# e-c-k-e-r/tortoise-tts

Hardware: AMD Instinct MI355X
Metric: audio-sec/wall-sec (RTF^-1), 16 AR candidates x 80 DDIM steps (higher is better)
Workload: dtype bf16; 1 GPU; configs[1]: 1 utterance/GPU, 64 text tokens, 16 AR candidates x 250 mel tokens (KV-cached decode), latent pass on 16 candidates, 80 DDIM steps with cond-free guidance at T=1088 (11.6 s audio); candidates=16, ddim_steps=80, mel_frames=1088, parallelism=single GPU, small_models=False, vocoder_in_step=False

## Files before the change

tortoise_tts_amd/csrc/ar.hip:

```cpp
#include "ttk_common.h"
#include "ttk_conv.h"

using namespace ttk;

namespace {

struct ARLayer {
	float *ln1_g, *ln1_b, *ln2_g, *ln2_b;
	Mat attn, proj, fc, proj2;
};

__global__ void k_build_prefill_emb(const float* cond, int Bc, const int64_t* text, int Tt, int B, int d,
									const float* text_emb, const float* text_pos, const float* mel_emb, const float* mel_pos,
									int start_text, int stop_text, int start_mel, float* out, const int64_t* prompt = nullptr, int prompt_rows = 0, int n_in = 0) {
	const int S = Tt + 4 + n_in;
	const int64_t idx = (int64_t)blockIdx.x * blockDim.x + threadIdx.x;
	const int d4 = d / 4;
	if (idx >= (int64_t)B * S * d4) return;
	const int c = (int)(idx % d4) * 4;
	const int64_t row = idx / d4;
	const int b = (int)(row / S), s = (int)(row - (int64_t)b * S);
	float4 v;
	if (s == 0) {
		v = *(const float4*)(cond + (int64_t)(Bc == 1 ? 0 : b) * d + c);
// ... 1 lines not shown
		const int j = s - (Tt + 3);
		const int64_t tok = j == 0 ? start_mel : prompt[(int64_t)(prompt_rows == 1 ? 0 : b) * n_in + j - 1];
		const float4 e = *(const float4*)(mel_emb + tok * d + c), w = *(const float4*)(mel_pos + (int64_t)j * d + c);
		v = make_float4(e.x + w.x, e.y + w.y, e.z + w.z, e.w + w.w);
	} else {
		const int j = s - 1;
		const int64_t tok = j == 0 ? start_text : (j == Tt + 1 ? stop_text : text[j - 1]);
		const float4 e = *(const float4*)(text_emb + tok * d + c), w = *(const float4*)(text_pos + (int64_t)j * d + c);
		v = make_float4(e.x + w.x, e.y + w.y, e.z + w.z, e.w + w.w);
	}
	*(float4*)(out + row * d + c) = v;
}

__global__ void k_build_latent_emb(const float* cond, const int64_t* text, int Tt, const int64_t* codes, int M, int B, int d,
								   const float* text_emb, const float* text_pos, const float* mel_emb, const float* mel_pos,
								   int start_text, int stop_text, int start_mel, int stop_mel, float* out) {
	const int S = Tt + M + 5;
	const int64_t idx = (int64_t)blockIdx.x * blockDim.x + threadIdx.x;
	const int d4 = d / 4;
	if (idx >= (int64_t)B * S * d4) return;
	const int c = (int)(idx % d4) * 4;
	const int64_t row = idx / d4;
	const int b = (int)(row / S), s = (int)(row - (int64_t)b * S);
	float4 v;
	if (s == 0) {
		v = *(const float4*)(cond + (int64_t)b * d + c);
	} else if (s < Tt + 3) {
		const int j = s - 1;
		const int64_t tok = j == 0 ? start_text : (j == Tt + 1 ? stop_text : text[(int64_t)b * Tt + j - 1]);
		const float4 e = *(const float4*)(text_emb + tok * d + c), w = *(const float4*)(text_pos + (int64_t)j * d + c);
		v = make_float4(e.x + w.x, e.y + w.y, e.z + w.z, e.w + w.w);
	} else {
		const int j = s - (Tt + 3);
		const int64_t tok = j == 0 ? start_mel : (j == M + 1 ? stop_mel : codes[(int64_t)b * M + j - 1]);
		const float4 e = *(const float4*)(mel_emb + tok * d + c), w = *(const float4*)(mel_pos + (int64_t)j * d + c);
		v = make_float4(e.x + w.x, e.y + w.y, e.z + w.z, e.w + w.w);
	}
	*(float4*)(out + row * d + c) = v;
}

__global__ void k_build_score_targets(const int64_t* text, int Tt, int stop_text, const int64_t* codes, int M, int stop_mel, int B, int64_t* tgt_text, int64_t* tgt_mel) {
	const int64_t idx = (int64_t)blockIdx.x * blockDim.x + threadIdx.x;
	const int64_t nt = (int64_t)B * (Tt + 2), nm = (int64_t)B * (M + 2);
	if (idx < nt) {
		const int b = (int)(idx / (Tt + 2)), j = (int)(idx - (int64_t)b * (Tt + 2));
		tgt_text[idx] = j < Tt ? text[(int64_t)b * Tt + j] : stop_text;
	} else if (idx < nt + nm) {
		const int64_t i = idx - nt;
		const int b = (int)(i / (M + 2)), j = (int)(i - (int64_t)b * (M + 2));
		tgt_mel[i] = j < M ? codes[(int64_t)b * M + j] : stop_mel;
	}
}

// ... 21 lines not shown
	void *attn_out, *hbuf;
	void* x_frag = nullptr;
	int poison = 0;
	int frag_rows = 0;
	int shared_rows = 0;
	const int64_t* rng_args = nullptr; const int64_t* rng_draws = nullptr; float* rng_q = nullptr;
	int* d_health = nullptr;
	float* ring_base = nullptr; const int64_t* ring_idx = nullptr; int64_t ring_stride = 0;
	int64_t* d_ring = nullptr;
	int lnfold = 1;
	int lean = 1;
	WsBuf ws_x, ws_a, ws_qkv, ws_ao, ws_h;
	WsBuf ws_score;
	int B = 0, P = 0, k = 0, ready = 0;
	int Pmax = 0;
	~ttk_ar() { attn_pos_slot_release(pos_slot); }
};

static int poison_scratch(ttk_ar* h, hipStream_t s) {
	if (!h->poison) return TTK_OK;
	for (WsBuf* w : {&h->ws_x, &h->ws_a, &h->ws_qkv, &h->ws_ao, &h->ws_h, &h->ws_score})
		if (w->p) TTK_HIP(hipMemsetAsync(w->p, 0xFF, w->cap, s));
	return TTK_OK;
}

static int dense_forward(ttk_ar* h, float* x, int B, int S, bool write_kv, hipStream_t s, int kv_row0 = 0, int kv_t0 = 0) {
	const int d = h->cfg.model_dim, H = h->cfg.heads, dt = h->dt;
	const int rows = B * S;
	TTK_TRY(h->ws_a.reserve((size_t)rows * d * h->es));
	TTK_TRY(h->ws_qkv.reserve((size_t)rows * 3 * d * h->es));
	TTK_TRY(h->ws_ao.reserve((size_t)rows * d * h->es));
	TTK_TRY(h->ws_h.reserve((size_t)rows * 4 * d * h->es));
	for (int l = 0; l < h->cfg.layers; ++l) {
		const ARLayer& L = h->L[l];
		launch_layernorm(dt, x, d, rows, d, L.ln1_g, L.ln1_b, nullptr, nullptr, h->ws_a.p, d, 0, s);
		launch_gemm(dt, dense_gemm(h->ws_a.p, d, L.attn, rows, h->ws_qkv.p, 0), s);
		if (write_kv) {
			const size_t row0 = (size_t)kv_row0 * H * h->cfg.max_ctx * 64;
			char* kc = (char*)h->kc + ((size_t)l * h->kv_layer_stride + row0) * h->es;
			char* vc = (char*)h->vc + ((size_t)l * h->kv_layer_stride + row0) * h->es;
			launch_kv_scatter(dt, h->ws_qkv.p, B, S, H, kc, vc, h->cfg.max_ctx, s, kv_t0);
		}
		AttnParams a = {};
		a.qkv = h->ws_qkv.p; a.ld = 3 * d; a.q_off = 0; a.k_off = d; a.v_off = 2 * d; a.head_stride = 64;
		a.out = h->ws_ao.p; a.ldo = d; a.nb = B; a.T = S; a.H = H; a.causal = 1; a.bias = nullptr; a.scale = 0.125f;
		launch_attn_fwd(dt, a, s);
		gemm_plain(dt, h->ws_ao.p, d, L.proj, rows, x, x, 1, s);
		launch_layernorm(dt, x, d, rows, d, L.ln2_g, L.ln2_b, nullptr, nullptr, h->ws_a.p, d, 0, s);
		GemmParams fc = dense_gemm(h->ws_a.p, d, L.fc, rows, h->ws_h.p, 0);
		fc.act = ACT_GELU_NEW;
		launch_gemm(dt, fc, s);
		gemm_plain(dt, h->ws_h.p, 4 * d, L.proj2, rows, x, x, 1, s);
	}
	return TTK_OK;
}

namespace ttk {

int skinny_waves(int role, bool ln_prologue, int dt, int d) {
	if (d < 1024 || role == DR_HEAD) return 4;
	if (ln_prologue || dt == DT_F32) return 8;
// ... 71 lines not shown
		TTK_TRY(decode_launch(ctx, proj, B, s));
		DecodeLaunch fc = {DR_FC, &L.fc, 4 * d, d, h->x_frag, L.ln2_g, L.ln2_b};
		fc.out_T = h->hbuf; fc.x = h->x; fc.ldx = d;
		TTK_TRY(decode_launch(ctx, fc, B, s));
		DecodeLaunch proj2 = {DR_PROJ2, &L.proj2, d, 4 * d, h->hbuf};
		proj2.out_f32 = h->x; proj2.out_T = xf;
		TTK_TRY(decode_launch(ctx, proj2, B, s));
	}
	if (h->ring_base && !hidden_out) launch_layernorm(dt, h->x, d, B, d, h->lnf_g, h->lnf_b, h->fn_g, h->fn_b, h->attn_out, d, 0, s, 1, nullptr, h->ring_idx, h->ring_stride, h->d_ring);
	else launch_layernorm(dt, h->x, d, B, d, h->lnf_g, h->lnf_b, h->fn_g, h->fn_b, h->attn_out, d, 0, s, 1, hidden_out);
	DecodeLaunch head = {DR_HEAD, &h->head, c.number_mel_codes, d, h->attn_out};
	head.out_f32 = logits_out; head.bump = true; head.d_pos = h->d_pos;
	return decode_launch(ctx, head, B, s);
}

extern "C" {

int ttk_ar_create(ttk_ar** out, const ttk_ar_config* cfg, const ttk_weight_view* w, int n_w) {
	TTK_REQUIRE(out && cfg && w, TTK_E_ARG, "ttk_ar_create: null argument");
	TTK_REQUIRE(cfg->model_dim % 64 == 0 && cfg->heads * 64 == cfg->model_dim, TTK_E_ARG,
				"ttk_ar_create: head_dim must be 64 (model_dim %d, heads %d)", cfg->model_dim, cfg->heads);
	TTK_REQUIRE(cfg->model_dim <= 2048, TTK_E_ARG, "ttk_ar_create: model_dim %d > 2048 unsupported", cfg->model_dim);
	TTK_REQUIRE(cfg->dtype == TTK_F32 || cfg->dtype == TTK_BF16 || cfg->dtype == TTK_F16 || cfg->dtype == TTK_FP8W, TTK_E_ARG, "ttk_ar_create: bad dtype %d", cfg->dtype);
	TTK_REQUIRE(cfg->max_batch >= 1 && cfg->max_batch <= (cfg->dtype == TTK_F32 ? 32 : 64), TTK_E_ARG,
				"ttk_ar_create: max_batch %d out of range", cfg->max_batch);
	TTK_REQUIRE(cfg->max_ctx >= 8, TTK_E_ARG, "ttk_ar_create: max_ctx %d too small", cfg->max_ctx);
	{
		const int kdt = kernel_dtype(cfg->dtype), d = cfg->model_dim;
		for (int B = 1; B <= cfg->max_batch; ++B) {
			const int mt = decode_row_tiles(B);
// ... 64 lines not shown
	for (int B = 1; B <= cfg->max_batch; ++B)
		if (16 * decode_row_tiles(B) > h->frag_rows) { set_error("ttk_ar_create: %d rows would request %d fragment rows, %d allocated", B, 16 * decode_row_tiles(B), h->frag_rows); return TTK_E_STATE; }
	TTK_TRY(h->arena.alloc(&h->attn_out, frag_rows * d * h->es));
	if (hipMemset(h->attn_out, 0, frag_rows * d * h->es) != hipSuccess) return TTK_E_HIP;
	TTK_TRY(h->arena.alloc(&h->hbuf, frag_rows * 4 * d * h->es));
	if (hipMemset(h->hbuf, 0, frag_rows * 4 * d * h->es) != hipSuccess) return TTK_E_HIP;
	TTK_TRY(h->arena.alloc(&h->x_frag, frag_rows * d * h->es));
	if (hipMemset(h->x_frag, 0, frag_rows * d * h->es) != hipSuccess) return TTK_E_HIP;
	{
		const char* ep = getenv("TTK_DEBUG_POISON");
		h->poison = ep && atoi(ep) != 0;
		const char* el = getenv("TTK_AR_LNFOLD");
		h->lnfold = el ? (atoi(el) != 0) : 1;
		const char* eg = getenv("TTK_AR_LEAN");
		h->lean = eg ? (atoi(eg) != 0) : 1;
	}
	hipError_t e = hipDeviceSynchronize();
	if (e != hipSuccess) { set_error("ttk_ar_create: %s", hipGetErrorString(e)); return TTK_E_HIP; }
	*out = h.release();
	return TTK_OK;
}

int ttk_ar_destroy(ttk_ar* h) {
	if (!h) return TTK_OK;
	(void)hipDeviceSynchronize();
	delete h;
	return TTK_OK;
}

static int prefill_impl(ttk_ar* h, const float* cond_latent, int Bc, const int64_t* text, int Tt, const int64_t* prompt, int prompt_rows, int n_in, int B, float* logits_out,
						void* stream, const char* who) {
	TTK_REQUIRE(h && cond_latent && text && logits_out, TTK_E_ARG, "%s: null argument", who);
	const ttk_ar_config& c = h->cfg;
	TTK_REQUIRE(B >= 1 && B <= c.max_batch, TTK_E_ARG, "%s: B=%d exceeds max_batch=%d", who, B, c.max_batch);
	TTK_REQUIRE(Bc == 1 || Bc == B, TTK_E_ARG, "%s: cond batch %d must be 1 or B=%d", who, Bc, B);
	TTK_REQUIRE(Tt >= 1 && Tt + 2 <= c.max_text_seq_len, TTK_E_ARG, "%s: %d text tokens exceed the position table (%d)", who, Tt, c.max_text_seq_len - 2);
	TTK_REQUIRE(n_in == 0 || (prompt && (prompt_rows == 1 || prompt_rows == B)), TTK_E_ARG, "%s: %d prompt tokens need 1 or B=%d prompt rows (got %d)", who, n_in, B, prompt_rows);
	TTK_REQUIRE(n_in >= 0 && n_in + 2 < c.max_mel_seq_len, TTK_E_ARG, "%s: %d prompt tokens exceed the mel position table (%d)", who, n_in, c.max_mel_seq_len);
	const int S = Tt + 4 + n_in, d = c.model_dim;
	TTK_REQUIRE(S + 1 <= c.max_ctx, TTK_E_ARG, "%s: prefix of %d rows does not fit max_ctx=%d", who, S, c.max_ctx);
	hipStream_t s = (hipStream_t)stream;
	const bool shared = Bc == 1 && B > 1 && (n_in == 0 || prompt_rows == 1);
	const int Bp = shared ? 1 : B;
	TTK_TRY(h->ws_x.reserve((size_t)Bp * S * d * sizeof(float)));
	float* x = (float*)h->ws_x.p;
	const int64_t total = (int64_t)Bp * S * (d / 4);
	hipLaunchKernelGGL(k_build_prefill_emb, dim3(grid_for(total)), dim3(256), 0, s, cond_latent, Bc, text, Tt, Bp, d,
					   h->text_emb, h->text_pos, h->mel_emb, h->mel_pos, c.start_text_token, c.stop_text_token, c.start_mel_token, x, prompt, prompt_rows, n_in);
	TTK_TRY(dense_forward(h, x, Bp, S, true, s));
	launch_copy_rows(x + (size_t)(S - 1) * d, shared ? 0 : (int64_t)S * d, h->x, d, B, d, s);
	TTK_TRY(head_launch(h, B, logits_out, s));
	launch_set_int(h->d_pos, S, s);
	launch_set_int(h->d_pos + 1, shared ? S : 0, s);
	TTK_TRY(poison_scratch(h, s));
	h->B = B; h->P = h->Pmax = Tt + 3; h->k = n_in; h->ready = 1; h->lines_mode = 0;
	h->shared_rows = shared ? S : 0;
	TTK_HIP(hipGetLastError());
	return TTK_OK;
}

int ttk_ar_prefill(ttk_ar* h, const float* cond_latent, int Bc, const int64_t* text, int Tt, int B, float* logits_out, void* stream) {
	return prefill_impl(h, cond_latent, Bc, text, Tt, nullptr, 0, 0, B, logits_out, stream, "ttk_ar_prefill");
}

int ttk_ar_prefill_prompted(ttk_ar* h, const float* cond_latent, int Bc, const int64_t* text, int Tt, const int64_t* prompt, int prompt_rows, int n_prompt, int B,
							float* logits_out, void* stream) {
	TTK_REQUIRE(n_prompt >= 1 && prompt, TTK_E_ARG, "ttk_ar_prefill_prompted: needs at least one prompt token");
	return prefill_impl(h, cond_latent, Bc, text, Tt, prompt, prompt_rows, n_prompt, B, logits_out, stream, "ttk_ar_prefill_prompted");
}

int ttk_ar_prefill_lines(ttk_ar* h, const float* cond_latents, const int64_t* text, const int* text_len, int n_lines, int rows_per_line,
						 float* logits_out, void* stream) {
	TTK_REQUIRE(h && cond_latents && text && text_len && logits_out, TTK_E_ARG, "ttk_ar_prefill_lines: null argument");
	const ttk_ar_config& c = h->cfg;
	const int B = n_lines * rows_per_line, d = c.model_dim;
	TTK_REQUIRE(n_lines >= 1 && rows_per_line >= 1 && B <= c.max_batch, TTK_E_ARG, "ttk_ar_prefill_lines: %d lines x %d candidates exceed max_batch=%d", n_lines, rows_per_line, c.max_batch);
	int Smax = 0;
	for (int g = 0; g < n_lines; ++g) {
		const int Tt = text_len[g];
		TTK_REQUIRE(Tt >= 1 && Tt + 2 <= c.max_text_seq_len, TTK_E_ARG, "ttk_ar_prefill_lines: line %d: %d text tokens exceed the position table (%d)", g, Tt, c.max_text_seq_len - 2);
		TTK_REQUIRE(Tt + 5 <= c.max_ctx, TTK_E_ARG, "ttk_ar_prefill_lines: line %d: prefix of %d rows does not fit max_ctx=%d", g, Tt + 4, c.max_ctx);
		Smax = Tt + 4 > Smax ? Tt + 4 : Smax;
	}
	hipStream_t s = (hipStream_t)stream;
	TTK_TRY(h->ws_x.reserve((size_t)Smax * d * sizeof(float)));
	float* x = (float*)h->ws_x.p;
	int64_t toff = 0;
	for (int g = 0; g < n_lines; ++g) {
		const int Tt = text_len[g], S = Tt + 4, r0 = g * rows_per_line, start = Smax - S;
		const int64_t total = (int64_t)S * (d / 4);
		hipLaunchKernelGGL(k_build_prefill_emb, dim3(grid_for(total)), dim3(256), 0, s, cond_latents + (size_t)g * d, 1, text + toff, Tt, 1, d,
						   h->text_emb, h->text_pos, h->mel_emb, h->mel_pos, c.start_text_token, c.stop_text_token, c.start_mel_token, x);
		TTK_TRY(dense_forward(h, x, 1, S, true, s, r0, start));
		launch_copy_rows(x + (size_t)(S - 1) * d, 0, h->x + (size_t)r0 * d, d, rows_per_line, d, s);
		launch_fill_int2((int*)(h->d_rowinfo + r0), start, r0, rows_per_line, s);
		toff += Tt;
	}
	TTK_TRY(head_launch(h, B, logits_out, s));
	launch_set_int(h->d_pos, Smax, s);
// ... 33 lines not shown
}

int ttk_ar_sample_next(ttk_ar* h, const ttk_sample_args* a, void* stream) {
	TTK_REQUIRE(h && a, TTK_E_ARG, "ttk_ar_sample_next: null argument");
	TTK_REQUIRE(h->ready, TTK_E_STATE, "ttk_ar_sample_next: call ttk_ar_prefill first");
	TTK_REQUIRE(a->B == h->B && a->V == h->cfg.number_mel_codes, TTK_E_ARG, "ttk_ar_sample_next: shape (B %d, V %d) is not the prefilled one (B %d, V %d)",
				a->B, a->V, h->B, h->cfg.number_mel_codes);
	return launch_sample_step(a, h->mel_emb, h->mel_pos, h->x, h->cfg.model_dim, h->cfg.max_mel_seq_len, h->lnfold ? h->x_frag : nullptr, elem_kind(h->dt),
							  (hipStream_t)stream, "ttk_ar_sample_next");
}

int ttk_ar_reorder_cache(ttk_ar* h, const int64_t* beam_idx, void* stream) {
	TTK_REQUIRE(h && beam_idx, TTK_E_ARG, "ttk_ar_reorder_cache: null argument");
	TTK_REQUIRE(h->ready, TTK_E_STATE, "ttk_ar_reorder_cache: call ttk_ar_prefill first");
	TTK_REQUIRE(!h->lines_mode, TTK_E_STATE, "ttk_ar_reorder_cache: the candidates of a line batch (ttk_ar_prefill_lines) keep their own histories");
	return launch_kv_reorder(h->kc, h->vc, h->cfg.layers, h->cfg.max_batch, h->cfg.heads, h->cfg.max_ctx, h->es, h->d_pos, beam_idx, h->B, (hipStream_t)stream,
							 "ttk_ar_reorder_cache");
}

int ttk_ar_set_noise(ttk_ar* h, const int64_t* rng_args, const int64_t* draws, float* q) {
	TTK_REQUIRE(h, TTK_E_ARG, "ttk_ar_set_noise: null handle");
	TTK_REQUIRE((rng_args && draws && q) || (!rng_args && !draws && !q), TTK_E_ARG, "ttk_ar_set_noise: pass all three pointers or none");
	h->rng_args = rng_args; h->rng_draws = draws; h->rng_q = q;
	return TTK_OK;
}

int ttk_ar_set_hidden_ring(ttk_ar* h, float* base, const int64_t* index, int64_t stride, void* stream) {
	TTK_REQUIRE(h, TTK_E_ARG, "ttk_ar_set_hidden_ring: null handle");
	TTK_REQUIRE(!base || (index && stride >= 0), TTK_E_ARG, "ttk_ar_set_hidden_ring: a ring needs its device index and a stride");
	h->ring_base = base; h->ring_idx = base ? index : nullptr; h->ring_stride = base ? stride : 0;
// ... 31 lines not shown
	TTK_REQUIRE(h->ready, TTK_E_STATE, "ttk_ar_last_hidden: call ttk_ar_prefill first");
	const int d = h->cfg.model_dim;
	launch_layernorm(h->dt, h->x, d, h->B, d, h->lnf_g, h->lnf_b, h->fn_g, h->fn_b, hidden_out, d, 1, (hipStream_t)stream);
	TTK_HIP(hipGetLastError());
	return TTK_OK;
}

int ttk_ar_latents(ttk_ar* h, const float* cond, const int64_t* text, int Tt, const int64_t* codes, int M, int B, float* latents_out, void* stream) {
	TTK_REQUIRE(h && cond && text && codes && latents_out, TTK_E_ARG, "ttk_ar_latents: null argument");
	const ttk_ar_config& c = h->cfg;
	TTK_REQUIRE(B >= 1 && Tt >= 1 && M >= 1, TTK_E_ARG, "ttk_ar_latents: empty input (B=%d Tt=%d M=%d)", B, Tt, M);
	TTK_REQUIRE(Tt + 2 <= c.max_text_seq_len, TTK_E_ARG, "ttk_ar_latents: %d text tokens exceed the position table", Tt);
	TTK_REQUIRE(M + 2 <= c.max_mel_seq_len, TTK_E_ARG, "ttk_ar_latents: %d mel codes exceed the position table (%d)", M, c.max_mel_seq_len - 2);
	const int S = Tt + M + 5, d = c.model_dim;
	hipStream_t s = (hipStream_t)stream;
	TTK_TRY(h->ws_x.reserve((size_t)B * S * d * sizeof(float)));
	float* x = (float*)h->ws_x.p;
	const int64_t total = (int64_t)B * S * (d / 4);
	hipLaunchKernelGGL(k_build_latent_emb, dim3(grid_for(total)), dim3(256), 0, s, cond, text, Tt, codes, M, B, d,
					   h->text_emb, h->text_pos, h->mel_emb, h->mel_pos, c.start_text_token, c.stop_text_token, c.start_mel_token, c.stop_mel_token, x);
	TTK_TRY(dense_forward(h, x, B, S, false, s));
	for (int b = 0; b < B; ++b)
		launch_layernorm(h->dt, x + ((size_t)b * S + Tt + 3) * d, d, M, d, h->lnf_g, h->lnf_b, h->fn_g, h->fn_b,
						 latents_out + (size_t)b * M * d, d, 1, s);
	TTK_TRY(poison_scratch(h, s));
	TTK_HIP(hipGetLastError());
	return TTK_OK;
}

int ttk_ar_score(ttk_ar* h, const float* cond, const int64_t* text, int Tt, const int64_t* codes, int M, int B, float* loss_out, float* nll_text_out, float* nll_mel_out,
// ... 49 lines not shown
```

tortoise_tts_amd/csrc/attn.hip:

```cpp
#include <hip/hip_ext.h>

#include <mutex>
#include "ttk_common.h"
#include "ttk_kernels.h"

namespace ttk {

#ifndef TTK_ATTN_XCD_MAP
#define TTK_ATTN_XCD_MAP 1
#endif
constexpr int HD = 64;
constexpr float NEG_BIG = -1e30f;
constexpr float LOG2E = 1.4426950408889634f;

template <typename T> struct VT;
template <> struct VT<bf16> {
	static __device__ __forceinline__ bf16x8 load(const char* Vs, int kb, int d0, int lane) {
		const int i = lane & 15, g = lane >> 4;
		const int q = i >> 2, p = i & 3;
		const int col = d0 + 4 * p;
		const int r0 = kb + 4 * g + q, r1 = r0 + 16;
		const int ch = col >> 3, sub = (col & 7) * 2;
		typedef __attribute__((address_space(3))) bf16x4 lds_v4;
		const bf16x4 lo = __builtin_amdgcn_ds_read_tr16_b64_v4bf16((lds_v4*)(Vs + r0 * 128 + ((ch ^ (r0 & 7)) << 4) + sub));
// ... 18 lines not shown
};
template <> struct VT<float> {
	static __device__ __forceinline__ f32x8 load(const char* Vs, int kb, int d0, int lane) {
		const int i = lane & 15, g = lane >> 4;
		const int col = d0 + i;
		f32x8 r;
#pragma unroll
		for (int j = 0; j < 8; ++j) {
			const int row = kb + 4 * g + (j & 3) + (j >> 2) * 16;
			r[j] = *(const float*)(Vs + row * 256 + (((col >> 2) ^ (row & 15)) << 4) + (col & 3) * 4);
		}
		return r;
	}
};

template <typename T, bool CAUSAL, bool BIAS, int QT, int NWV = 4>
__global__ __launch_bounds__(64 * NWV, NWV == 4 ? 2 : 1) void k_attn_fwd(AttnParams p) {
	constexpr bool BAL = NWV == 9;
	typedef typename Frag<T>::type FragT;
	constexpr int ES = sizeof(T);
	constexpr int ROWB = HD * ES;
	constexpr int NCH = ROWB / 16;
	constexpr int SWM = NCH - 1;
	constexpr int FCH = 8 * ES / 16;
	constexpr int TILE_CH = 64 * NCH;
	constexpr int NTH = BAL ? 512 : 64 * NWV;
	constexpr int CPT = TILE_CH / NTH;
	__shared__ __attribute__((aligned(16))) char Ks[64 * ROWB];
	__shared__ __attribute__((aligned(16))) char Vs[64 * ROWB];
	__shared__ float bias_s[132];
	__shared__ float band_s[BIAS ? 288 : 4];

	const int tid = threadIdx.x, lane = tid & 63, wave = tid >> 6;
	int bx = blockIdx.x, h = blockIdx.y, b = blockIdx.z;
	if (BAL && TTK_ATTN_XCD_MAP && ((gridDim.y * gridDim.z) & 7) == 0) {
		const int L = (blockIdx.z * gridDim.y + blockIdx.y) * gridDim.x + blockIdx.x, G = gridDim.x;
		const int xcd = L & 7, sidx = L >> 3, bh = (sidx / G) * 8 + xcd;
		bx = sidx - (sidx / G) * G; h = bh % (int)gridDim.y; b = bh / (int)gridDim.y;
	}
	constexpr int QW = 16 * QT, QB = NWV * QW;
	const int li = lane & 15, g = lane >> 4;
	TTK_WSTAMP(p.stamps, (blockIdx.z * gridDim.y + blockIdx.y) * gridDim.x + blockIdx.x, 0);
	const int TL = p.tlen ? p.tlen[b] : p.T;
	int q0 = bx * QB + wave * QW;
	int cnt = NWV;
	if (BAL) {
		const int tiles = (TL + 15) / 16, G = gridDim.x, per = tiles / G, extra = tiles - per * G;
		cnt = per + (bx < extra ? 1 : 0);
		q0 = 16 * (bx * per + min(bx, extra) + wave);
		if (cnt == 0) return;
	} else if (bx * QB >= TL) return;
	const T* base = (const T*)p.qkv + (int64_t)b * p.T * p.ld;
	const int qc = p.q_off + h * p.head_stride, kc = p.k_off + h * p.head_stride, vc = p.v_off + h * p.head_stride;

	__shared__ unsigned pf_sink[64 * NWV];
	if (p.pf) {
		const int lin = (blockIdx.z * gridDim.y + blockIdx.y) * gridDim.x + blockIdx.x;
		l2_touch_for_next(p.pf, p.pf_bytes, p.pf_taps, __builtin_amdgcn_readfirstlane(lds_byte_addr(pf_sink) + (threadIdx.x >> 6) * 256), lin, gridDim.x * gridDim.y * gridDim.z, threadIdx.x, 64 * NWV);
	}
	if (BIAS) {
		if (tid < 129) bias_s[tid] = p.bias[h * 129 + tid] * LOG2E;
		for (int i = tid; i < 288; i += 64 * NWV) { const int rel = i - 144; band_s[i] = p.bias[h * 129 + (rel < -64 ? -64 : (rel > 64 ? 64 : rel)) + 64] * LOG2E; }
	}

	auto load_q = [&](int qt, int ks) -> FragT {
		int row = q0 + 16 * qt + li;
		row = row < TL ? row : TL - 1;
		const FragT f = *(const FragT*)(base + (int64_t)row * p.ld + qc + 32 * ks + 8 * g);
		FragT o;
#pragma unroll
		for (int j = 0; j < 8; ++j) o[j] = cvt<T>((float)f[j] * p.scale);
		return o;
	};
	const FragT q00 = load_q(0, 0), q01 = load_q(0, 1), q10 = load_q(QT - 1, 0), q11 = load_q(QT - 1, 1);

	f32x4 o[QT][4];
	float m_run[QT], l_run[QT];
#pragma unroll
	for (int qt = 0; qt < QT; ++qt) {
		m_run[qt] = NEG_BIG; l_run[qt] = 0.f;
#pragma unroll
		for (int dt = 0; dt < 4; ++dt) o[qt][dt] = f32x4{0.f, 0.f, 0.f, 0.f};
	}

	int nkt = (TL + 63) / 64;
	if (CAUSAL) { const int last_q = min(bx * QB + QB - 1, TL - 1); nkt = min(nkt, last_q / 64 + 1); }

	uint4 rk0, rk1, rk2, rk3, rv0, rv1, rv2, rv3;
	rk1 = rv1 = rk2 = rk3 = rv2 = rv3 = make_uint4(0, 0, 0, 0);
	auto thr_ptr = [&](int i) -> const T* { const int id = tid + NTH * i; return base + (int64_t)(id / NCH) * p.ld + (id % NCH) * (16 / ES); };
	const T* const sp0 = thr_ptr(0);
	const T* const sp1 = thr_ptr(CPT > 1 ? 1 : 0);
	const T* const sp2 = thr_ptr(CPT > 2 ? 2 : 0);
	const T* const sp3 = thr_ptr(CPT > 2 ? 3 : 0);
	const int64_t tile_step = (int64_t)64 * p.ld;
	auto ld1 = [&](int kt, int i, uint4& k, uint4& v) {
		const T* src;
		if (kt * 64 + 64 <= TL) {
			src = (i == 0 ? sp0 : (i == 1 ? sp1 : (i == 2 ? sp2 : sp3))) + kt * tile_step;
		} else {
			const int id = tid + NTH * i, row = id / NCH, c = id % NCH;
			int key = kt * 64 + row;
			key = key < TL ? key : TL - 1;
			src = base + (int64_t)key * p.ld + c * (16 / ES);
		}
		k = *(const uint4*)(src + kc);
		v = *(const uint4*)(src + vc);
	};
	auto st1 = [&](int i, const uint4& k, const uint4& v) {
		const int id = tid + NTH * i, row = id / NCH, c = id % NCH;
		const int off = row * ROWB + ((c ^ (row & SWM)) << 4);
		*(uint4*)(Ks + off) = k;
// ... 29 lines not shown
#if !(defined(TTK_DIAG_ATTN) && (TTK_DIAG_ATTN & 1))
		__syncthreads();
#endif
#if defined(TTK_DIAG_ATTN) && (TTK_DIAG_ATTN & 2)
		if (kt == 0)
#endif
		store_kv();
#if !(defined(TTK_DIAG_ATTN) && (TTK_DIAG_ATTN & 1))
		__syncthreads();
#endif
#if !(defined(TTK_DIAG_ATTN) && (TTK_DIAG_ATTN & 2))
		load_kv(kt + 1 < nkt ? kt + 1 : kt);
#endif

		const int k0 = kt * 64;
		const bool wave_active = (!CAUSAL || k0 <= q0 + QW - 1) && (!BAL || wave < cnt);
		TTK_PH_MARK(ph_sync_, k0);
		if (wave_active) {
			f32x4 s[QT][4];
#pragma unroll
			for (int qt = 0; qt < QT; ++qt)
#pragma unroll
				for (int nt = 0; nt < 4; ++nt) s[qt][nt] = f32x4{0.f, 0.f, 0.f, 0.f};
#pragma unroll
			for (int ks = 0; ks < 2; ++ks) {
#pragma unroll
				for (int nt = 0; nt < 4; ++nt) {
					union { FragT v; uint4 q[FCH]; } kf;
					const int row = 16 * nt + li;
					const int c0 = (32 * ks + 8 * g) * ES / 16;
#pragma unroll
// ... 101 lines not shown
	}
#endif

#ifdef TTK_CLOCK_STAMPS
	if (p.stamps && lane == 0) {
		unsigned long long* st_ = p.stamps + ((size_t)((blockIdx.z * gridDim.y + blockIdx.y) * gridDim.x + blockIdx.x) * 16 + (threadIdx.x >> 6)) * 8;
		st_[6] = ((__builtin_amdgcn_s_memtime() - clk0_) << 32) | ((__builtin_amdgcn_s_memrealtime() - rt0_) & 0xffffffffull);
	}
#endif
#pragma unroll
	for (int qt = 0; qt < QT; ++qt) {
		float l = l_run[qt];
		l = fold32_add(fold16_add(l));
		const float inv = 1.0f / l;
		const int qi = q0 + 16 * qt + li;
		if (qi < TL && (!BAL || wave < cnt)) {
			if (p.out_f8) {
				unsigned char* dst = (unsigned char*)p.out + ((int64_t)b * p.T + qi) * p.ldo + h * HD;
#pragma unroll
				for (int dt = 0; dt < 4; ++dt)
					*(unsigned*)(dst + 16 * dt + 4 * g) = pack4_fp8(o[qt][dt][0] * inv, o[qt][dt][1] * inv, o[qt][dt][2] * inv, o[qt][dt][3] * inv);
			} else {
				T* dst = (T*)p.out + ((int64_t)b * p.T + qi) * p.ldo + h * HD;
#pragma unroll
				for (int dt = 0; dt < 4; ++dt)
#pragma unroll
					for (int r = 0; r < 4; ++r) dst[16 * dt + 4 * g + r] = cvt<T>(o[qt][dt][r] * inv);
			}
		}
	}
	TTK_WSTAMPD(p.stamps, (blockIdx.z * gridDim.y + blockIdx.y) * gridDim.x + blockIdx.x, 4, o[0][0][0]);
#if defined(TTK_STAMPS) && TTK_STAMPS == 2
	asm volatile("s_waitcnt vmcnt(0)" ::: "memory");
	TTK_WSTAMP(p.stamps, (blockIdx.z * gridDim.y + blockIdx.y) * gridDim.x + blockIdx.x, 5);
#endif
}

struct AttnBalanced { int G, tiles; const char* refusal; };
static AttnBalanced attn_balanced(const AttnParams& p) {
	const int tiles = (p.T + 15) / 16;
	if (p.causal || p.tlen) return {0, tiles, "form 4 (balanced) is non-causal and takes no tlen (a workgroup's tile share is computed from T)"};
	if ((int64_t)p.nb * p.H > 256 || 256 % (p.nb * p.H) != 0) return {0, tiles, "form 4 (balanced) needs 256 % (nb * H) == 0"};
	const int G = 256 / (p.nb * p.H);
	if ((tiles + G - 1) / G > 9) return {G, tiles, "form 4 (balanced) has 9 waves: at most 9 16-query tiles per workgroup, ceil(ceil(T / 16) / (256 / (nb * H))) <= 9"};
	return {G, tiles, nullptr};
}
const char* attn_fwd_form_refusal(const AttnParams& p, int form) {
	if (form < 0 || form > 4) return "form must be 0 (the launcher's choice), 1 (64-query blocks), 2 (128-query blocks), 3 (8 waves x 16 queries) or 4 (balanced)";
	if (form == 3 && p.causal) return "form 3 (8 waves x 16 queries) has no causal kernel";
	return form == 4 ? attn_balanced(p).refusal : nullptr;
}
static int attn_fwd_choice(const AttnParams& p) {
	const AttnBalanced b = attn_balanced(p);
	if (!b.refusal && b.tiles / b.G >= 6) return 4;
	return (int64_t)((p.T + 127) / 128) * p.H * p.nb >= 512 ? 2 : 1;
}
template <typename T, int QT, int NWV>
static void attn_fwd_go(const AttnParams& p, int gx, hipStream_t s) {
	const dim3 grid(gx, p.H, p.nb), block(64 * NWV);
	if constexpr (NWV == 4) {
		if (p.causal) { hipLaunchKernelGGL((k_attn_fwd<T, true, false, QT, NWV>), grid, block, 0, s, p); return; }
	}
	if (p.bias) hipLaunchKernelGGL((k_attn_fwd<T, false, true, QT, NWV>), grid, block, 0, s, p);
	else hipLaunchKernelGGL((k_attn_fwd<T, false, false, QT, NWV>), grid, block, 0, s, p);
}
void launch_attn_fwd(int dt, const AttnParams& p, hipStream_t s, int form) {
	ProfScope prof(PROF_ATTN_FWD, 4.0 * p.nb * p.H * (double)p.T * p.T * HD * (p.causal ? 0.5 : 1.0), s);
	if (form == 0) form = attn_fwd_choice(p);
	by_dtype(dt, [&](auto t) {
		using T = decltype(t);
		if (form == 1) attn_fwd_go<T, 1, 4>(p, (p.T + 63) / 64, s);
		else if (form == 2) attn_fwd_go<T, 2, 4>(p, (p.T + 127) / 128, s);
		else if (form == 3) attn_fwd_go<T, 1, 8>(p, (p.T + 127) / 128, s);
		else attn_fwd_go<T, 1, 9>(p, 256 / (p.nb * p.H), s);
	});
}

__device__ __forceinline__ int64_t decode_out_index(const AttnDecodeParams& p, int b, int h, int e) {
	if (!p.out_frag) return ((int64_t)b * p.H + h) * HD + e;
	const int n = h * HD + e;
	return TTK_FRAG_INDEX(b, n, p.H * HD / 32);
}

__device__ __attribute__((aligned(64))) int g_pos_line[16];
static unsigned g_pos_slots_used = 0;
static std::mutex g_pos_slots_mutex;
int attn_pos_slot_acquire(int** words_out) {
// ... 170 lines not shown
```

tortoise_tts_amd/csrc/ttk_kernels.h:

```cpp
#pragma once
#include <hip/hip_runtime.h>
#include <stdint.h>

namespace ttk {

enum DType { DT_F32 = 0, DT_BF16 = 1, DT_FP8W = 2, DT_FP8 = 3, DT_F16 = 4 };
inline int elem_kind(int dt) { return dt == DT_F32 ? 1 : (dt == DT_F16 ? 2 : 0); }
inline size_t dtype_size(int dt) { return dt == DT_F32 ? 4 : 2; }
inline int kernel_dtype(int dt) { return (dt == DT_FP8W || dt == DT_FP8) ? DT_BF16 : dt; }
template <typename F>
auto by_dtype(int dt, F f) {
	if (dt == DT_BF16) return f(__bf16());
	if (dt == DT_F16) return f(_Float16());
	return f(float());
}
template <typename F>
auto by_f32_bf16(int dt, F f) { return dt == DT_BF16 ? f(__bf16()) : f(float()); }
inline unsigned grid_for(int64_t total) { return (unsigned)((total + 255) / 256); }

enum ProfKind { PROF_GEMM = 0, PROF_SKINNY = 1, PROF_ATTN_FWD = 2, PROF_ATTN_DECODE = 3, PROF_GN_STATS = 4, PROF_GN_APPLY = 5,
				PROF_LAYERNORM = 6, PROF_KINDS = 7 };
extern bool g_prof_on;
void prof_start(int kind, double work, hipStream_t s);
void prof_stop(hipStream_t s);
// ... 122 lines not shown

struct AttnParams {
	const void* qkv; int64_t ld;
	int q_off, k_off, v_off, head_stride;
	void* out; int64_t ldo;
	int out_f8;
	int nb, T, H, causal;
	const int* tlen;
	const float* bias;
	float scale;
	const void* pf; int64_t pf_bytes; int pf_taps;
#ifdef TTK_STAMPS
	unsigned long long* stamps;
#endif
};
void launch_attn_fwd(int dt, const AttnParams& p, hipStream_t s, int form = 0);
const char* attn_fwd_form_refusal(const AttnParams& p, int form);

struct AttnDecodeParams {
	const float* qbuf;
	const void* kcache; const void* vcache;
	const int* d_pos;
	int B, H, max_ctx;
	int ctx_hint;
	void* out;
	int out_frag;
	const int2* row_info;
	int pos_slot_p1;
	int shared_rows;
#ifdef TTK_STAMPS
	unsigned long long* stamps;
// ... 45 lines not shown
```

Baseline: 40.60 audio-sec/wall-sec.

## Reuse prefill KV cache for the shared text prefix in the latent pass

The latent pass no longer recomputes the conditioning and text prefix. When the last prefill was a shared, unprompted one and an on-device check confirms the conditioning and text are unchanged, the pass runs the transformer only on rows from a 16-aligned prefix boundary onward. Causal attention reads the prefix keys and values straight from the decode KV cache through a new prefix variant of the forward attention kernel. In exchange it adds a host-blocking stream synchronize for the match check, and it falls back to the full path under graph capture or after a cache reorder.

New measurement: 40.69 audio-sec/wall-sec (median of 4 runs). About the same (+0.2%).

```diff
diff --git a/tortoise_tts_amd/csrc/ar.hip b/tortoise_tts_amd/csrc/ar.hip
--- a/tortoise_tts_amd/csrc/ar.hip
+++ b/tortoise_tts_amd/csrc/ar.hip
@@ -39,14 +39,14 @@
 
 __global__ void k_build_latent_emb(const float* cond, const int64_t* text, int Tt, const int64_t* codes, int M, int B, int d,
 								   const float* text_emb, const float* text_pos, const float* mel_emb, const float* mel_pos,
-								   int start_text, int stop_text, int start_mel, int stop_mel, float* out) {
-	const int S = Tt + M + 5;
+								   int start_text, int stop_text, int start_mel, int stop_mel, float* out, int s0 = 0) {
+	const int S = Tt + M + 5 - s0;
 	const int64_t idx = (int64_t)blockIdx.x * blockDim.x + threadIdx.x;
 	const int d4 = d / 4;
 	if (idx >= (int64_t)B * S * d4) return;
 	const int c = (int)(idx % d4) * 4;
 	const int64_t row = idx / d4;
-	const int b = (int)(row / S), s = (int)(row - (int64_t)b * S);
+	const int b = (int)(row / S), s = s0 + (int)(row - (int64_t)b * S);
 	float4 v;
 	if (s == 0) {
 		v = *(const float4*)(cond + (int64_t)b * d + c);
@@ -62,6 +62,20 @@
 		v = make_float4(e.x + w.x, e.y + w.y, e.z + w.z, e.w + w.w);
 	}
 	*(float4*)(out + row * d + c) = v;
+}
+
+__global__ void k_save_prefix(const float* cond, const int64_t* text, int Tt, int d, float* cond_out, int64_t* text_out) {
+	const int i = blockIdx.x * blockDim.x + threadIdx.x;
+	if (i < d) cond_out[i] = cond[i];
+	else if (i < d + Tt) text_out[i - d] = text[i - d];
+}
+
+__global__ __launch_bounds__(1024) void k_match_prefix(const float* cond, const int64_t* text, int Tt, int B, int d, const float* cond_saved, const int64_t* text_saved, int* match) {
+	int diff = 0;
+	for (int64_t i = threadIdx.x; i < (int64_t)B * d; i += blockDim.x) diff |= __float_as_uint(cond[i]) != __float_as_uint(cond_saved[i % d]);
+	for (int64_t i = threadIdx.x; i < (int64_t)B * Tt; i += blockDim.x) diff |= text[i] != text_saved[i % Tt];
+	diff = __syncthreads_or(diff);
+	if (threadIdx.x == 0) *match = diff ? 0 : 1;
 }
 
 __global__ void k_build_score_targets(const int64_t* text, int Tt, int stop_text, const int64_t* codes, int M, int stop_mel, int B, int64_t* tgt_text, int64_t* tgt_mel) {
@@ -113,7 +127,15 @@
 	WsBuf ws_score;
 	int B = 0, P = 0, k = 0, ready = 0;
 	int Pmax = 0;
-	~ttk_ar() { attn_pos_slot_release(pos_slot); }
+	int latent_prefix = 1;
+	int prefix_rows = 0;
+	const char* prefix_why = "the handle was never prefilled";
+	float* pfx_cond = nullptr; int64_t* pfx_text = nullptr;
+	int* pfx_match = nullptr;
+	~ttk_ar() {
+		attn_pos_slot_release(pos_slot);
+		if (pfx_match) (void)hipHostFree(pfx_match);
+	}
 };
 
 static int poison_scratch(ttk_ar* h, hipStream_t s) {
@@ -123,7 +145,7 @@
 	return TTK_OK;
 }
 
-static int dense_forward(ttk_ar* h, float* x, int B, int S, bool write_kv, hipStream_t s, int kv_row0 = 0, int kv_t0 = 0) {
+static int dense_forward(ttk_ar* h, float* x, int B, int S, bool write_kv, hipStream_t s, int kv_row0 = 0, int kv_t0 = 0, int pfx_rows = -1) {
 	const int d = h->cfg.model_dim, H = h->cfg.heads, dt = h->dt;
 	const int rows = B * S;
 	TTK_TRY(h->ws_a.reserve((size_t)rows * d * h->es));
@@ -143,7 +165,11 @@
 		AttnParams a = {};
 		a.qkv = h->ws_qkv.p; a.ld = 3 * d; a.q_off = 0; a.k_off = d; a.v_off = 2 * d; a.head_stride = 64;
 		a.out = h->ws_ao.p; a.ldo = d; a.nb = B; a.T = S; a.H = H; a.causal = 1; a.bias = nullptr; a.scale = 0.125f;
-		launch_attn_fwd(dt, a, s);
+		if (pfx_rows >= 0) {
+			const size_t layer = (size_t)l * h->kv_layer_stride * h->es;
+			const AttnPrefix pfx = {pfx_rows, (const char*)h->kc + layer, (const char*)h->vc + layer, (int64_t)h->cfg.max_ctx * 64, 0};
+			launch_attn_fwd(dt, a, s, 0, &pfx);
+		} else launch_attn_fwd(dt, a, s);
 		gemm_plain(dt, h->ws_ao.p, d, L.proj, rows, x, x, 1, s);
 		launch_layernorm(dt, x, d, rows, d, L.ln2_g, L.ln2_b, nullptr, nullptr, h->ws_a.p, d, 0, s);
 		GemmParams fc = dense_gemm(h->ws_a.p, d, L.fc, rows, h->ws_h.p, 0);
@@ -245,6 +271,43 @@
 	return decode_launch(ctx, head, B, s);
 }
 
+static int latents_on_cached_prefix(ttk_ar* h, const float* cond, const int64_t* text, int Tt, const int64_t* codes, int M, int B, float* latents_out, hipStream_t s, int* taken) {
+	const ttk_ar_config& c = h->cfg;
+	const int d = c.model_dim;
+	*taken = 0;
+	const char* why = h->prefix_why;
+	if (!why && h->prefix_rows != Tt + 3) why = "the prefilled text has another length (Tt)";
+	if (!why && B > c.max_batch) why = "B exceeds the handle's max_batch";
+	if (!why) {
+		hipStreamCaptureStatus cs = hipStreamCaptureStatusNone;
+		if (hipStreamIsCapturing(s, &cs) != hipSuccess) { (void)hipGetLastError(); why = "the stream's capture status cannot be read"; }
+		else if (cs != hipStreamCaptureStatusNone) why = "the stream is being captured";
+	}
+	if (!why) {
+		*(volatile int*)h->pfx_match = 0;
+		hipLaunchKernelGGL(k_match_prefix, dim3(1), dim3(1024), 0, s, cond, text, Tt, B, d, h->pfx_cond, h->pfx_text, h->pfx_match);
+		TTK_HIP(hipStreamSynchronize(s));
+		if (!*(volatile int*)h->pfx_match) why = "a conditioning row or a text line is not the prefilled one";
+	}
+	if (why) {
+		TTK_REQUIRE(h->latent_prefix != 2, TTK_E_STATE, "ttk_ar_latents: TTK_AR_LATENT_PREFIX=require, but the prefix in the decode cache cannot be used: %s", why);
+		return TTK_OK;
+	}
+	const int P = Tt + 3, P0 = P & ~15, R = Tt + M + 5 - P0;
+	TTK_TRY(h->ws_x.reserve((size_t)B * R * d * sizeof(float)));
+	float* x = (float*)h->ws_x.p;
+	const int64_t total = (int64_t)B * R * (d / 4);
+	hipLaunchKernelGGL(k_build_latent_emb, dim3(grid_for(total)), dim3(256), 0, s, cond, text, Tt, codes, M, B, d,
+					   h->text_emb, h->text_pos, h->mel_emb, h->mel_pos, c.start_text_token, c.stop_text_token, c.start_mel_token, c.stop_mel_token, x, P0);
+	TTK_TRY(dense_forward(h, x, B, R, false, s, 0, 0, P0));
+	for (int b = 0; b < B; ++b)
+		launch_layernorm(h->dt, x + ((size_t)b * R + P - P0) * d, d, M, d, h->lnf_g, h->lnf_b, h->fn_g, h->fn_b, latents_out + (size_t)b * M * d, d, 1, s);
+	TTK_TRY(poison_scratch(h, s));
+	TTK_HIP(hipGetLastError());
+	*taken = 1;
+	return TTK_OK;
+}
+
 extern "C" {
 
 int ttk_ar_create(ttk_ar** out, const ttk_ar_config* cfg, const ttk_weight_view* w, int n_w) {
@@ -339,7 +402,13 @@
 		h->lnfold = el ? (atoi(el) != 0) : 1;
 		const char* eg = getenv("TTK_AR_LEAN");
 		h->lean = eg ? (atoi(eg) != 0) : 1;
-	}
+		const char* ex = getenv("TTK_AR_LATENT_PREFIX");
+		h->latent_prefix = !ex ? 1 : (strcmp(ex, "require") == 0 ? 2 : (atoi(ex) != 0));
+	}
+	TTK_TRY(h->arena.alloc((void**)&h->pfx_cond, (size_t)d * sizeof(float)));
+	TTK_TRY(h->arena.alloc((void**)&h->pfx_text, (size_t)cfg->max_text_seq_len * sizeof(int64_t)));
+	TTK_HIP(hipHostMalloc((void**)&h->pfx_match, sizeof(int), hipHostMallocDefault));
+	*h->pfx_match = 0;
 	hipError_t e = hipDeviceSynchronize();
 	if (e != hipSuccess) { set_error("ttk_ar_create: %s", hipGetErrorString(e)); return TTK_E_HIP; }
 	*out = h.release();
@@ -367,12 +436,15 @@
 	hipStream_t s = (hipStream_t)stream;
 	const bool shared = Bc == 1 && B > 1 && (n_in == 0 || prompt_rows == 1);
 	const int Bp = shared ? 1 : B;
+	h->prefix_why = "the last prefill did not finish";
 	TTK_TRY(h->ws_x.reserve((size_t)Bp * S * d * sizeof(float)));
 	float* x = (float*)h->ws_x.p;
 	const int64_t total = (int64_t)Bp * S * (d / 4);
 	hipLaunchKernelGGL(k_build_prefill_emb, dim3(grid_for(total)), dim3(256), 0, s, cond_latent, Bc, text, Tt, Bp, d,
 					   h->text_emb, h->text_pos, h->mel_emb, h->mel_pos, c.start_text_token, c.stop_text_token, c.start_mel_token, x, prompt, prompt_rows, n_in);
 	TTK_TRY(dense_forward(h, x, Bp, S, true, s));
+	const char* why = Bc != 1 ? "the last prefill had one conditioning latent per candidate" : (n_in != 0 ? "the last prefill was a prompted one (ttk_ar_prefill_prompted)" : nullptr);
+	if (!why) hipLaunchKernelGGL(k_save_prefix, dim3(grid_for(d + Tt)), dim3(256), 0, s, cond_latent, text, Tt, d, h->pfx_cond, h->pfx_text);
 	launch_copy_rows(x + (size_t)(S - 1) * d, shared ? 0 : (int64_t)S * d, h->x, d, B, d, s);
 	TTK_TRY(head_launch(h, B, logits_out, s));
 	launch_set_int(h->d_pos, S, s);
@@ -381,6 +453,7 @@
 	h->B = B; h->P = h->Pmax = Tt + 3; h->k = n_in; h->ready = 1; h->lines_mode = 0;
 	h->shared_rows = shared ? S : 0;
 	TTK_HIP(hipGetLastError());
+	h->prefix_rows = Tt + 3; h->prefix_why = why;
 	return TTK_OK;
 }
 
@@ -408,6 +481,7 @@
 		Smax = Tt + 4 > Smax ? Tt + 4 : Smax;
 	}
 	hipStream_t s = (hipStream_t)stream;
+	h->prefix_why = "the last prefill was a line batch (ttk_ar_prefill_lines): its prefixes are right-aligned in several slices";
 	TTK_TRY(h->ws_x.reserve((size_t)Smax * d * sizeof(float)));
 	float* x = (float*)h->ws_x.p;
 	int64_t toff = 0;
@@ -471,6 +545,7 @@
 	TTK_REQUIRE(h && beam_idx, TTK_E_ARG, "ttk_ar_reorder_cache: null argument");
 	TTK_REQUIRE(h->ready, TTK_E_STATE, "ttk_ar_reorder_cache: call ttk_ar_prefill first");
 	TTK_REQUIRE(!h->lines_mode, TTK_E_STATE, "ttk_ar_reorder_cache: the candidates of a line batch (ttk_ar_prefill_lines) keep their own histories");
+	h->prefix_why = "the cache was reordered (ttk_ar_reorder_cache) since the last prefill";
 	return launch_kv_reorder(h->kc, h->vc, h->cfg.layers, h->cfg.max_batch, h->cfg.heads, h->cfg.max_ctx, h->es, h->d_pos, beam_idx, h->B, (hipStream_t)stream,
 							 "ttk_ar_reorder_cache");
 }
@@ -532,6 +607,11 @@
 	TTK_REQUIRE(M + 2 <= c.max_mel_seq_len, TTK_E_ARG, "ttk_ar_latents: %d mel codes exceed the position table (%d)", M, c.max_mel_seq_len - 2);
 	const int S = Tt + M + 5, d = c.model_dim;
 	hipStream_t s = (hipStream_t)stream;
+	if (h->latent_prefix) {
+		int fast = 0;
+		const int r = latents_on_cached_prefix(h, cond, text, Tt, codes, M, B, latents_out, s, &fast);
+		if (r != TTK_OK || fast) return r;
+	}
 	TTK_TRY(h->ws_x.reserve((size_t)B * S * d * sizeof(float)));
 	float* x = (float*)h->ws_x.p;
 	const int64_t total = (int64_t)B * S * (d / 4);
diff --git a/tortoise_tts_amd/csrc/attn.hip b/tortoise_tts_amd/csrc/attn.hip
--- a/tortoise_tts_amd/csrc/attn.hip
+++ b/tortoise_tts_amd/csrc/attn.hip
@@ -1,6 +1,7 @@
 #include <hip/hip_ext.h>
 
 #include <mutex>
+#include <type_traits>
 #include "ttk_common.h"
 #include "ttk_kernels.h"
 
@@ -56,9 +57,11 @@
 	}
 };
 
-template <typename T, bool CAUSAL, bool BIAS, int QT, int NWV = 4>
-__global__ __launch_bounds__(64 * NWV, NWV == 4 ? 2 : 1) void k_attn_fwd(AttnParams p) {
+template <typename T, bool CAUSAL, bool BIAS, int QT, int NWV = 4, typename P = AttnParams>
+__global__ __launch_bounds__(64 * NWV, NWV == 4 ? 2 : 1) void k_attn_fwd(P p) {
 	constexpr bool BAL = NWV == 9;
+	constexpr bool PFX = std::is_same<P, AttnParamsPfx>::value;
+	static_assert(!PFX || (CAUSAL && !BIAS && NWV == 4), "the prefix form is causal, without bias, on the 4-wave kernels");
 	typedef typename Frag<T>::type FragT;
 	constexpr int ES = sizeof(T);
 	constexpr int ROWB = HD * ES;
@@ -81,9 +84,11 @@
 		bx = sidx - (sidx / G) * G; h = bh % (int)gridDim.y; b = bh / (int)gridDim.y;
 	}
 	constexpr int QW = 16 * QT, QB = NWV * QW;
+	const int P0 = [&] { if constexpr (PFX) return p.x.rows; else return 0; }();
+	if (PFX) bx += P0 / QB;
 	const int li = lane & 15, g = lane >> 4;
 	TTK_WSTAMP(p.stamps, (blockIdx.z * gridDim.y + blockIdx.y) * gridDim.x + blockIdx.x, 0);
-	const int TL = p.tlen ? p.tlen[b] : p.T;
+	const int TL = (p.tlen ? p.tlen[b] : p.T) + P0;
 	int q0 = bx * QB + wave * QW;
 	int cnt = NWV;
 	if (BAL) {
@@ -108,6 +113,7 @@
 	auto load_q = [&](int qt, int ks) -> FragT {
 		int row = q0 + 16 * qt + li;
 		row = row < TL ? row : TL - 1;
+		if (PFX) row = (row > P0 ? row : P0) - P0;
 		const FragT f = *(const FragT*)(base + (int64_t)row * p.ld + qc + 32 * ks + 8 * g);
 		FragT o;
 #pragma unroll
@@ -138,6 +144,21 @@
 	const int64_t tile_step = (int64_t)64 * p.ld;
 	auto ld1 = [&](int kt, int i, uint4& k, uint4& v) {
 		const T* src;
+		if constexpr (PFX) {
+			const int id = tid + NTH * i, row = id / NCH, c = id % NCH;
+			int key = kt * 64 + row;
+			key = key < TL ? key : TL - 1;
+			if (key < P0) {
+				const int64_t off = (int64_t)b * p.x.seq_stride + (int64_t)h * p.x.head_stride + (int64_t)key * HD + c * (16 / ES);
+				k = *(const uint4*)((const T*)p.x.k + off);
+				v = *(const uint4*)((const T*)p.x.v + off);
+			} else {
+				src = base + (int64_t)(key - P0) * p.ld + c * (16 / ES);
+				k = *(const uint4*)(src + kc);
+				v = *(const uint4*)(src + vc);
+			}
+			return;
+		}
 		if (kt * 64 + 64 <= TL) {
 			src = (i == 0 ? sp0 : (i == 1 ? sp1 : (i == 2 ? sp2 : sp3))) + kt * tile_step;
 		} else {
@@ -197,7 +218,7 @@
 #endif
 
 		const int k0 = kt * 64;
-		const bool wave_active = (!CAUSAL || k0 <= q0 + QW - 1) && (!BAL || wave < cnt);
+		const bool wave_active = (!CAUSAL || k0 <= q0 + QW - 1) && (!BAL || wave < cnt) && (!PFX || q0 + QW > P0);
 		TTK_PH_MARK(ph_sync_, k0);
 		if (wave_active) {
 			f32x4 s[QT][4];
@@ -329,14 +350,14 @@
 		l = fold32_add(fold16_add(l));
 		const float inv = 1.0f / l;
 		const int qi = q0 + 16 * qt + li;
-		if (qi < TL && (!BAL || wave < cnt)) {
+		if (qi < TL && (!BAL || wave < cnt) && (!PFX || qi >= P0)) {
 			if (p.out_f8) {
-				unsigned char* dst = (unsigned char*)p.out + ((int64_t)b * p.T + qi) * p.ldo + h * HD;
+				unsigned char* dst = (unsigned char*)p.out + ((int64_t)b * p.T + qi - P0) * p.ldo + h * HD;
 #pragma unroll
 				for (int dt = 0; dt < 4; ++dt)
 					*(unsigned*)(dst + 16 * dt + 4 * g) = pack4_fp8(o[qt][dt][0] * inv, o[qt][dt][1] * inv, o[qt][dt][2] * inv, o[qt][dt][3] * inv);
 			} else {
-				T* dst = (T*)p.out + ((int64_t)b * p.T + qi) * p.ldo + h * HD;
+				T* dst = (T*)p.out + ((int64_t)b * p.T + qi - P0) * p.ldo + h * HD;
 #pragma unroll
 				for (int dt = 0; dt < 4; ++dt)
 #pragma unroll
@@ -365,27 +386,38 @@
 	if (form == 3 && p.causal) return "form 3 (8 waves x 16 queries) has no causal kernel";
 	return form == 4 ? attn_balanced(p).refusal : nullptr;
 }
-static int attn_fwd_choice(const AttnParams& p) {
+static int attn_fwd_blocks(const AttnParams& p, int QB, const AttnPrefix* pfx) {
+	const int P0 = pfx ? pfx->rows : 0;
+	return (P0 + p.T + QB - 1) / QB - P0 / QB;
+}
+static int attn_fwd_choice(const AttnParams& p, const AttnPrefix* pfx) {
 	const AttnBalanced b = attn_balanced(p);
 	if (!b.refusal && b.tiles / b.G >= 6) return 4;
-	return (int64_t)((p.T + 127) / 128) * p.H * p.nb >= 512 ? 2 : 1;
+	return (int64_t)attn_fwd_blocks(p, 128, pfx) * p.H * p.nb >= 512 ? 2 : 1;
 }
 template <typename T, int QT, int NWV>
-static void attn_fwd_go(const AttnParams& p, int gx, hipStream_t s) {
+static void attn_fwd_go(const AttnParams& p, int gx, hipStream_t s, const AttnPrefix* pfx = nullptr) {
 	const dim3 grid(gx, p.H, p.nb), block(64 * NWV);
 	if constexpr (NWV == 4) {
+		if (p.causal && pfx) {
+			AttnParamsPfx px;
+			(AttnParams&)px = p; px.x = *pfx;
+			hipLaunchKernelGGL((k_attn_fwd<T, true, false, QT, NWV, AttnParamsPfx>), grid, block, 0, s, px);
+			return;
+		}
 		if (p.causal) { hipLaunchKernelGGL((k_attn_fwd<T, true, false, QT, NWV>), grid, block, 0, s, p); return; }
 	}
 	if (p.bias) hipLaunchKernelGGL((k_attn_fwd<T, false, true, QT, NWV>), grid, block, 0, s, p);
 	else hipLaunchKernelGGL((k_attn_fwd<T, false, false, QT, NWV>), grid, block, 0, s, p);
 }
-void launch_attn_fwd(int dt, const AttnParams& p, hipStream_t s, int form) {
-	ProfScope prof(PROF_ATTN_FWD, 4.0 * p.nb * p.H * (double)p.T * p.T * HD * (p.causal ? 0.5 : 1.0), s);
-	if (form == 0) form = attn_fwd_choice(p);
+void launch_attn_fwd(int dt, const AttnParams& p, hipStream_t s, int form, const AttnPrefix* pfx) {
+	const double keys = pfx ? p.T + 2.0 * pfx->rows : p.T;
+	ProfScope prof(PROF_ATTN_FWD, 4.0 * p.nb * p.H * (double)p.T * keys * HD * (p.causal ? 0.5 : 1.0), s);
+	if (form == 0) form = attn_fwd_choice(p, pfx);
 	by_dtype(dt, [&](auto t) {
 		using T = decltype(t);
-		if (form == 1) attn_fwd_go<T, 1, 4>(p, (p.T + 63) / 64, s);
-		else if (form == 2) attn_fwd_go<T, 2, 4>(p, (p.T + 127) / 128, s);
+		if (form == 1) attn_fwd_go<T, 1, 4>(p, attn_fwd_blocks(p, 64, pfx), s, pfx);
+		else if (form == 2) attn_fwd_go<T, 2, 4>(p, attn_fwd_blocks(p, 128, pfx), s, pfx);
 		else if (form == 3) attn_fwd_go<T, 1, 8>(p, (p.T + 127) / 128, s);
 		else attn_fwd_go<T, 1, 9>(p, 256 / (p.nb * p.H), s);
 	});
diff --git a/tortoise_tts_amd/csrc/ttk_kernels.h b/tortoise_tts_amd/csrc/ttk_kernels.h
--- a/tortoise_tts_amd/csrc/ttk_kernels.h
+++ b/tortoise_tts_amd/csrc/ttk_kernels.h
@@ -160,7 +160,12 @@
 	unsigned long long* stamps;
 #endif
 };
-void launch_attn_fwd(int dt, const AttnParams& p, hipStream_t s, int form = 0);
+struct AttnPrefix {
+	int rows;
+	const void* k; const void* v; int64_t head_stride, seq_stride;
+};
+struct AttnParamsPfx : AttnParams { AttnPrefix x; };
+void launch_attn_fwd(int dt, const AttnParams& p, hipStream_t s, int form = 0, const AttnPrefix* pfx = nullptr);
 const char* attn_fwd_form_refusal(const AttnParams& p, int form);
 
 struct AttnDecodeParams {
```
